# rohithr87/CILRS-Autonomous-Driving-CARLA

Measured on AMD Instinct MI355X. Metric: frames/sec CILRS train batch=128, higher is better.
Workload: dtype f32; 1 GPU; CILRS ResNet-34 train step (fwd+loss+bwd+Adam), Config A, 200x88 RGB, B=128/GPU, fp32; global_batch=128, parallelism=single

## Files before the change

### cilrs-autonomous-driving-carla_amd/cilrs_mi355/_lib.py

```python
from __future__ import annotations

import ctypes as C
import os

_HERE = os.path.dirname(os.path.abspath(__file__))
LIB_PATH = os.environ.get("CILRS_LIB") or os.path.join(_HERE, "libcilrs_hip.so")

c_float_p = C.POINTER(C.c_float)
vp = C.c_void_p
sz = C.c_size_t
i32 = C.c_int
i64 = C.c_int64
f32 = C.c_float
f64 = C.c_double
u64 = C.c_uint64


class Buffers(C.Structure):
    _fields_ = [("params", vp), ("grads", vp), ("bn_running", vp), ("bn_nbt", vp),
                ("workspace", vp)]


class AdamArgs(C.Structure):
    _fields_ = [("exp_avg", vp), ("exp_avg_sq", vp), ("lr", C.c_double), ("beta1", C.c_double),
# ... 112 lines not shown
                                         f32, vp, f32, vp]),
    "cilrs_swap": (i32, [vp, vp, sz, vp]),
    "cilrs_augment_u8": (i32, [vp, vp, i32, i32, i32, vp, vp, vp]),
    "cilrs_batch_assemble": (i32, [vp, i64, vp, vp, vp, vp, vp, i32, i32, i32, vp, vp, vp, vp, vp,
                                   vp]),
    "cilrs_eval_acc_doubles": (i32, []),
    "cilrs_eval_accumulate": (i32, [vp, vp, vp, vp, vp, i32, vp, vp, vp]),
    "cilrs_net_profile_enable": (i32, [vp, i32]),
    "cilrs_net_profile_collect": (i32, [vp]),
    "cilrs_net_profile_count": (i32, [vp]),
    "cilrs_net_profile_entry": (i32, [vp, i32, C.c_char_p, i32, C.POINTER(C.c_longlong),
                                      C.POINTER(f64), C.POINTER(f64), C.POINTER(f64)]),
    "cilrs_net_profile_reset": (i32, [vp]),
    "cilrs_conv2d_fwd": (i32, [vp, vp, vp] + [i32] * 11 + [vp, sz, vp]),
    "cilrs_conv2d_dgrad": (i32, [vp, vp, vp, vp] + [i32] * 11 + [vp, sz, vp]),
    "cilrs_conv2d_wgrad_scratch_floats": (sz, [i32] * 9),
    "cilrs_conv2d_wgrad": (i32, [vp, vp, vp, vp] + [i32] * 10 + [vp]),
    "cilrs_conv2d_16_scratch_halfs": (sz, [i32] * 8),
    "cilrs_conv2d_fwd_16": (i32, [vp, vp, vp, vp] + [i32] * 9 + [vp, vp]),
    "cilrs_conv2d_dgrad_16": (i32, [vp, vp, vp, vp] + [i32] * 9 + [vp, vp]),
    "cilrs_conv2d_wgrad_16_scratch_floats": (sz, [i32] * 8),
    "cilrs_conv2d_wgrad_16": (i32, [vp, vp, vp, vp] + [i32] * 9 + [vp, vp]),
    "cilrs_conv2d_train_16": (i32, [vp] * 9 + [i32, vp] + [i32] * 12 + [vp, vp]),
    "cilrs_conv2d_infer_16": (i32, [vp] * 5 + [i32] * 11 + [vp]),
    "cilrs_stem_fold_16": (i32, [vp, vp, vp, vp, i32, vp]),
    "cilrs_stem_infer_16": (i32, [vp, vp, vp, vp, i32, i32, i32, i32, vp]),
    "cilrs_maxpool_infer_16": (i32, [vp, vp, i32, i32, i32, i32, i32, vp]),
    "cilrs_avgpool_infer_16": (i32, [vp, vp, i32, i32, i32, i32, i32, vp]),
    "cilrs_bn16_train_fwd": (i32, [vp, i32, i32, vp, vp, vp, vp, vp, C.c_float, C.c_float, vp, i32,
                                   vp, vp, vp, i32, vp]),
# ... 70 lines not shown
```

### cilrs-autonomous-driving-carla_amd/csrc/common.h

```cpp
#pragma once
#include <hip/hip_runtime.h>
#include <stdint.h>
#include <stddef.h>
#include "../../include/cilrs_hip.h"

namespace cilrs {

typedef float f32x4 __attribute__((ext_vector_type(4)));
typedef float f32x16 __attribute__((ext_vector_type(16)));

void set_error(const char* fmt, ...);
const char* last_error();

#define CILRS_CHECK(cond, ...)                   \
    do {                                         \
        if (!(cond)) {                           \
            ::cilrs::set_error(__VA_ARGS__);     \
            return 1;                            \
        }                                        \
    } while (0)

#define CILRS_HIP(expr)                                                                 \
    do {                                                                                \
        hipError_t e_ = (expr);                                                         \
// ... 17 lines not shown
static inline int cdiv(int a, int b) { return (a + b - 1) / b; }

int device_cus();
int set_max_dynamic_lds(const void* kernel, int bytes);

constexpr float kImageMean[3] = {0.485f, 0.456f, 0.406f};
constexpr float kImageStd[3] = {0.229f, 0.224f, 0.225f};

#ifdef CILRS_EXPERIMENTS
int experiment_env(const char* name, int dflt);
#else
static inline int experiment_env(const char*, int dflt) { return dflt; }
#endif
static inline size_t cdivz(size_t a, size_t b) { return (a + b - 1) / b; }

struct ConvMulti {
    int n;
    int tile_begin[5];
    int Ho[4], Wo[4], out_h0[4], out_w0[4], ntaps[4];
    int tap_dh[4][4], tap_dw[4][4], tap_w[4][4];
};

struct ConvArgs {
    const float* x;
    const float* w;
    float* y;
    const float* addend;
    const float* bias;
    const float* ch_scale;
    const float* ch_shift;
    int relu_post;
    const float* mask;
    int N, H, W, Cin;
    int Ho, Wo, Cout;
    int KH, KW;
// ... 7 lines not shown
    int ntaps;
    int tap_dh[16], tap_dw[16], tap_w[16];
    float* bn_partial;
    int* bn_nblk;
    const float* bwd_z; const float* bwd_y; const float* bwd_stats; int bwd_relu;
    float* bwd_partial; int* bwd_nblk;
    float* scratch;
    size_t scratch_floats;
    int force_cfg;
    int force_splitk;
    int splitk;
    int prio_mode;
    ConvMulti multi;
};
int launch_conv_igemm(const ConvArgs& a, hipStream_t s);
int slab_reduce_rows(int M, int C, int* rows_per_block);
int launch_slab_reduce_cols(int mode, const float* slabs, int splits, float* y, const float* addend,
                            int M, int C, const float* bwd_z, const float* bwd_y,
                            const float* bwd_stats, int bwd_relu, float* partial, hipStream_t s);
struct DgradArgs {
    const float* dy; const float* w; float* dx; const float* addend;
    const float* mask; int mask_ld; float mask_scale;
    int N, H, W, Cin, Ho, Wo, Cout, K, stride, pad;
    int dy_ld, dx_ld;
    float* scratch; size_t scratch_floats; int force_cfg, force_splitk;
    const float* bwd_z; const float* bwd_y; const float* bwd_stats; int bwd_relu;
    float* bwd_partial; int* bwd_nblk;
};
int launch_conv_dgrad(const DgradArgs& a, hipStream_t s);

// ... 496 lines not shown
```

### cilrs-autonomous-driving-carla_amd/csrc/conv_igemm.hip

```cpp
#include "common.h"

#include <stdlib.h>
#include <string.h>

namespace cilrs {

namespace {

constexpr int BK = 32;
constexpr int APITCH = BK + 4;

__device__ float g_zero_page[64];

__device__ __forceinline__ int xcd_remap(int bid, int nwg) {
    const int q = nwg >> 3, r = nwg & 7, xcd = bid & 7;
    const int base = xcd < r ? xcd * (q + 1) : r * (q + 1) + (xcd - r) * q;
    return base + (bid >> 3);
}

#ifndef CILRS_IGEMM_DBG
#define CILRS_IGEMM_DBG 0
#endif
template <int BM, int BN, bool TAP_UNIFORM, bool DMA>
constexpr bool igemm_swz() { return DMA || (BM == 64 && BN == 64 && TAP_UNIFORM); }
// ... 15 lines not shown
    constexpr int JQ = BN / 4, BROWS = 256 / JQ;

    extern __shared__ __attribute__((aligned(16))) float smem[];
    float* As = smem;
    float* Bs = smem + NSTAGE * BM * APIT;

    const int tid = threadIdx.x;
    const int lane = tid & 63, wave = tid >> 6;
    const int l31 = lane & 31, lh = lane >> 5;
    const int wm = wave / WN, wn = wave % WN;

    wave_priority(a.prio_mode < 16 ? a.prio_mode : 0);
    wave_stagger(a.prio_mode);
    const int tilesN = a.Cout / BN;
    int logical = xcd_remap(blockIdx.x, gridDim.x);
    int cls = 0;
    int P_Ho = a.Ho, P_Wo = a.Wo, P_h0 = a.out_h0, P_w0 = a.out_w0, P_ntaps = a.ntaps;
    int M = M_, KT = KT_;
    if constexpr (MULTI) {
        while (cls + 1 < a.multi.n && logical >= a.multi.tile_begin[cls + 1]) ++cls;
        logical -= a.multi.tile_begin[cls];
        P_Ho = a.multi.Ho[cls]; P_Wo = a.multi.Wo[cls];
        P_h0 = a.multi.out_h0[cls]; P_w0 = a.multi.out_w0[cls];
        P_ntaps = a.multi.ntaps[cls];
        M = a.N * P_Ho * P_Wo;
        KT = P_ntaps * (a.Cin / BK);
    }
    auto tap_dh = [&](int t) { if constexpr (MULTI) return a.multi.tap_dh[cls][t]; else return a.tap_dh[t]; };
    auto tap_dw = [&](int t) { if constexpr (MULTI) return a.multi.tap_dw[cls][t]; else return a.tap_dw[t]; };
    auto tap_w = [&](int t) { if constexpr (MULTI) return a.multi.tap_w[cls][t]; else return a.tap_w[t]; };
    const int m0 = (logical / tilesN) * BM;
    const int n0 = (logical % tilesN) * BN;

    int kt_begin = 0, kt_end = KT;
    if (a.splitk > 1) {
        const int per = (KT + a.splitk - 1) / a.splitk;
        kt_begin = blockIdx.z * per;
        kt_end = min(KT, kt_begin + per);
    }
    const int nt = max(kt_end - kt_begin, 0);

    const int kq = tid & 7, r0 = tid >> 3;
    const int kql = DMA ? (kq ^ ((r0 >> 1) & 7)) : kq;
    long rowBase[A_PASSES];
    unsigned rowMask[A_PASSES];
    int rowH[A_PASSES], rowW[A_PASSES];
    const int HoWo = P_Ho * P_Wo;
#pragma unroll
    for (int i = 0; i < A_PASSES; ++i) {
        const int m = m0 + r0 + 32 * i;
        rowMask[i] = 0u; rowBase[i] = 0; rowH[i] = -(1 << 20); rowW[i] = 0;
        if (m < M) {
            const int n = m / HoWo, rem = m - n * HoWo;
// ... 307 lines not shown
            s1 += __shfl_xor(s1, 32);
            s2 += __shfl_xor(s2, 32);
            if (lh == 0) {
                red[(wm * BN + wn * WTN + j * 32 + l31) * 2] = s1;
                red[(wm * BN + wn * WTN + j * 32 + l31) * 2 + 1] = s2;
            }
        }
        __syncthreads();
        if (tid < BN) {
            float t1 = 0.f, t2 = 0.f;
#pragma unroll
            for (int w = 0; w < WM; ++w) {
                t1 += red[(w * BN + tid) * 2];
                t2 += red[(w * BN + tid) * 2 + 1];
            }
            const size_t mt = (size_t)(logical / tilesN), nmt = (size_t)((M + BM - 1) / BM);
            a.bn_partial[(size_t)(n0 + tid) * nmt + mt] = t1;
            a.bn_partial[(size_t)(a.Cout + n0 + tid) * nmt + mt] = t2;
        }
    }

    const bool partial = a.splitk > 1;
    const bool dense = (a.out_sh == 1) && (a.out_sw == 1) && (a.out_H == P_Ho) &&
                       (a.out_W == P_Wo);
    float* yout = partial ? a.y + (size_t)blockIdx.z * M * a.y_ld : a.y;
    const bool bwd_red = a.bwd_partial != nullptr && !partial;
    float bs1[TN], bs2[TN];
#pragma unroll
    for (int j = 0; j < TN; ++j) { bs1[j] = 0.f; bs2[j] = 0.f; }
#pragma unroll
    for (int i = 0; i < TM; ++i) {
#pragma unroll
        for (int j = 0; j < TN; ++j) {
            const int co = n0 + wn * WTN + j * 32 + l31;
            const int mbase = m0 + wm * WTM + i * 32 + 4 * lh;
            int pix[16];
#pragma unroll
            for (int r = 0; r < 16; ++r) {
                const int m = min(mbase + (r & 3) + 8 * (r >> 2), M - 1);
                if (dense || partial) {
                    pix[r] = m;
                } else {
                    const int n = m / HoWo, rem = m - n * HoWo;
                    const int oh = rem / P_Wo, ow = rem - oh * P_Wo;
                    pix[r] = (n * a.out_H + oh * a.out_sh + P_h0) * a.out_W +
                             ow * a.out_sw + P_w0;
                }
            }
            float v[16];
#pragma unroll
            for (int r = 0; r < 16; ++r) v[r] = acc[i][j][r];
            if (!partial) {
                if (a.ch_scale) {
                    const float sc = a.ch_scale[co], sh = a.ch_shift[co];
#pragma unroll
// ... 58 lines not shown
            float s1 = bs1[j] + __shfl_xor(bs1[j], 32);
            float s2 = bs2[j] + __shfl_xor(bs2[j], 32);
            if (lh == 0) {
                red[(wm * BN + wn * WTN + j * 32 + l31) * 2] = s1;
                red[(wm * BN + wn * WTN + j * 32 + l31) * 2 + 1] = s2;
            }
        }
        __syncthreads();
        if (tid < BN) {
            float t1 = 0.f, t2 = 0.f;
#pragma unroll
            for (int w = 0; w < WM; ++w) {
                t1 += red[(w * BN + tid) * 2];
                t2 += red[(w * BN + tid) * 2 + 1];
            }
            const size_t mt = (size_t)(logical / tilesN), nmt = (size_t)((M + BM - 1) / BM);
            a.bwd_partial[(size_t)(n0 + tid) * nmt + mt] = t1;
            a.bwd_partial[(size_t)(a.Cout + n0 + tid) * nmt + mt] = t2;
        }
    }
}

__device__ __forceinline__ int out_pixel(const ConvArgs& a, int m, int HoWo) {
    const int n = m / HoWo, rem = m - n * HoWo;
    const int oh = rem / a.Wo, ow = rem - oh * a.Wo;
    return (n * a.out_H + oh * a.out_sh + a.out_h0) * a.out_W + ow * a.out_sw + a.out_w0;
}

template <int MODE>
__global__ __launch_bounds__(256) void splitk_reduce_cols_kernel(const ConvArgs a,
                                                                 const float* __restrict__ part,
// ... 217 lines not shown
    CILRS_LAUNCH_CHECK();
    return 0;
}

struct Cfg { int bm, bn, occ; bool dma; float rate[5]; };
const Cfg kCfg[6] = {
    {128, 128, 2, false, {100.f, 113.f, 0.f, 0.f}},
    {128, 64, 2, false, {81.f, 100.f, 0.f, 0.f}},
    {64, 64, 5, false, {64.f, 90.f, 101.f, 108.f, 112.f}},
    {128, 128, 1, true, {125.f, 0.f, 0.f, 0.f}},
    {128, 64, 2, true, {110.f, 121.f, 0.f, 0.f}},
    {64, 64, 3, true, {94.f, 106.f, 111.f, 0.f}},
};
constexpr int kNumCfg = 6;

double cfg_cost(int M, int Cout, int KT, const Cfg& c, int splitk) {
    if (Cout % c.bn) return 1e30;
    const double blocks = (double)cdiv(M, c.bm) * (Cout / c.bn) * splitk;
    const long per_cu = (long)((blocks + 255) / 256);
    const double ktiles = (double)cdiv(KT, splitk);
    const double unit = 2.0 * c.bm * c.bn * BK * ktiles;
    const long full = per_cu / c.occ, rem = per_cu % c.occ;
    double t = 0.0;
    if (full) t += full * unit * 256.0 * c.occ / (c.rate[c.occ - 1] * 1e6);
    if (rem) t += unit * 256.0 * rem / (c.rate[rem - 1] * 1e6);
    t += (full + (rem ? 1 : 0)) * 2.5;
    if (splitk > 1) t += 3.0 + 0.12 * splitk + (double)M * Cout * 4.0 * (splitk + 1) / 3.0e6;
    return t;
}

struct Choice { int cfg; int splitk; };

Choice choose(int M, int Cout, int KT, bool allow_split, int force_cfg, int force_splitk) {
    static const int splits[11] = {1, 2, 3, 4, 6, 8, 12, 16, 24, 32, 48};
    static const int use_dma = experiment_env("CILRS_IGEMM_DMA", 0);
    Choice best{2, 1};
    double bc = 1e30;
    for (int c = 0; c < kNumCfg; ++c) {
        if (force_cfg >= 0 && c != force_cfg) continue;
        if (force_cfg < 0 && use_dma == 0 && kCfg[c].dma) continue;
        if (force_cfg < 0 && use_dma == 2 && !kCfg[c].dma) continue;
        for (int si = 0; si < 11; ++si) {
            int sk = splits[si];
            if (force_splitk > 0) {
                if (si > 0) break;
                sk = force_splitk;
            } else if (sk > 1 && (!allow_split || KT < 2 * sk)) {
                continue;
            }
            const double cost = cfg_cost(M, Cout, KT, kCfg[c], sk);
            if (cost < bc) { bc = cost; best = {c, sk}; }
        }
    }
    return best;
}

}

int launch_conv_igemm(const ConvArgs& a_in, hipStream_t s) {
    ConvArgs a = a_in;
    a.prio_mode = wave_priority_mode();
    const int M = a.N * a.Ho * a.Wo;
    const bool uniform = (a.Cin % BK) == 0;
    CILRS_CHECK(!uniform || ((size_t)a.N * a.H * a.W * a.x_ld * sizeof(float) < (1ull << 32) &&
                             (size_t)(a.w_mode == 0 ? a.Cout : a.Cin) * a.KH * a.KW *
                                     (a.w_mode == 0 ? a.Cin : a.w_cin) * sizeof(float) < (1ull << 32)),
                "conv_igemm: tensor larger than 4 GB");
    if (a.out_H == 0) {
        a.out_H = a.Ho; a.out_W = a.Wo; a.out_sh = a.out_sw = 1; a.out_h0 = a.out_w0 = 0;
    }
    if (uniform && a.ntaps == 0) {
        CILRS_CHECK(a.KH * a.KW <= 16, "conv_igemm: more than 16 taps on the uniform path");
        a.ntaps = a.KH * a.KW;
        for (int t = 0; t < a.ntaps; ++t) {
            a.tap_dh[t] = t / a.KW;
            a.tap_dw[t] = t % a.KW;
            a.tap_w[t] = (a.w_mode == 0) ? t : a.ntaps - 1 - t;
        }
    }
    const int KT = uniform ? a.ntaps * (a.Cin / BK) : cdiv(a.KH * a.KW * a.Cin, BK);
    const int Krow = a.KH * a.KW * a.Cin;
    CILRS_CHECK(a.Cout % 64 == 0, "conv_igemm: Cout=%d must be a multiple of 64", a.Cout);
    CILRS_CHECK(a.Cin % 4 == 0 && a.x_ld % 4 == 0 && a.y_ld % 4 == 0,
                "conv_igemm: Cin/x_ld/y_ld must be multiples of 4 (%d,%d,%d)", a.Cin, a.x_ld,
                a.y_ld);
    CILRS_CHECK(uniform || a.w_mode == 0, "conv_igemm: the generic-tap path is forward-only");
    CILRS_CHECK(a.w_mode == 0 || a.w_cin % 4 == 0, "conv_igemm: w_cin must be a multiple of 4");
    CILRS_CHECK(((uintptr_t)a.x & 15) == 0 && ((uintptr_t)a.w & 15) == 0 &&
                    ((uintptr_t)a.y & 15) == 0,
                "conv_igemm: pointers must be 16-byte aligned");
    CILRS_CHECK(M > 0 && (size_t)a.N * a.H * a.W < (1u << 31), "conv_igemm: bad M");
    CILRS_CHECK(a.ntaps <= 16, "conv_igemm: too many taps");

    const size_t slab = (size_t)M * a.y_ld;
    const bool can_split = a.scratch != nullptr && a.scratch_floats >= 2 * slab && uniform;
    Choice ch = choose(M, a.Cout, KT, can_split, a.force_cfg, a.force_splitk);
    while (ch.splitk > 1 && (size_t)ch.splitk * slab > a.scratch_floats) --ch.splitk;
    CILRS_CHECK(ch.splitk == 1 || (a.scratch && uniform), "conv_igemm: split-K needs scratch");
    CILRS_CHECK(ch.cfg >= 0 && ch.cfg < kNumCfg && a.Cout % kCfg[ch.cfg].bn == 0,
                "conv_igemm: tile config %d does not fit Cout=%d", ch.cfg, a.Cout);
    a.splitk = ch.splitk;
    const bool dense_out = a.out_sh == 1 && a.out_sw == 1 && a.out_H == a.Ho && a.out_W == a.Wo;
    const int tpr = a.Cout >> 2;
    const bool cols_ok = a.splitk > 1 && dense_out && a.Cout % 4 == 0 && tpr <= 256 &&
                         256 % tpr == 0 && a.y_ld % 4 == 0 && (!a.mask || a.mask_ld % 4 == 0);
    int cols_rows = 0, cols_nblk = 0;
    if (cols_ok && (a.bn_partial || a.bwd_partial)) {
        const int rpi = 256 / tpr;
        cols_rows = cdiv(cdiv(M, 1024), rpi) * rpi;
        cols_nblk = cdiv(M, cols_rows);
    }
    float* const fwd_partial = a.bn_partial;
    float* const bwd_partial = a.bwd_partial;
    if (a_in.bn_nblk)
        *a_in.bn_nblk = !a.bn_partial ? 0
                        : a.splitk == 1 ? cdiv(M, kCfg[ch.cfg].bm) : cols_nblk;
    if (!(a.splitk == 1 && dense_out)) a.bwd_partial = nullptr;
    if (a_in.bwd_nblk)
        *a_in.bwd_nblk = a.bwd_partial ? cdiv(M, kCfg[ch.cfg].bm) : (bwd_partial ? cols_nblk : 0);
    float* final_y = a.y;
    if (a.splitk > 1) a.y = a.scratch;

    int rc = 1;
#define CILRS_DISPATCH(BM_, BN_, DMA_)                                                          \
    do {                                                                                        \
        if (a.w_mode == 1) rc = launch_cfg<BM_, BN_, 2, 2, true, 1, DMA_>(a, M, Krow, KT, s);   \
        else if (uniform)  rc = launch_cfg<BM_, BN_, 2, 2, true, 0, DMA_>(a, M, Krow, KT, s);   \
        else               rc = launch_cfg<BM_, BN_, 2, 2, false, 0, DMA_>(a, M, Krow, KT, s);  \
    } while (0)
    switch (ch.cfg) {
        case 0: CILRS_DISPATCH(128, 128, false); break;
        case 1: CILRS_DISPATCH(128, 64, false); break;
        case 2: CILRS_DISPATCH(64, 64, false); break;
        case 3: CILRS_DISPATCH(128, 128, true); break;
        case 4: CILRS_DISPATCH(128, 64, true); break;
        default: CILRS_DISPATCH(64, 64, true); break;
    }
#undef CILRS_DISPATCH
// ... 103 lines not shown
        ConvMulti& mu = c.multi;
        memset(&mu, 0, sizeof(mu));
        mu.n = ncl;
        const int tilesN = c.Cout / 64;
        int total = 0;
        for (int i = 0; i < ncl; ++i) {
            mu.tile_begin[i] = total;
            total += cdiv(c.N * cl[i].Ho * cl[i].Wo, 64) * tilesN;
            mu.Ho[i] = cl[i].Ho; mu.Wo[i] = cl[i].Wo;
            mu.out_h0[i] = cl[i].ph; mu.out_w0[i] = cl[i].pw; mu.ntaps[i] = cl[i].nt;
            for (int t = 0; t < cl[i].nt; ++t) {
                mu.tap_dh[i][t] = cl[i].dh[t]; mu.tap_dw[i][t] = cl[i].dw[t];
                mu.tap_w[i][t] = cl[i].tw[t];
            }
        }
        for (int i = ncl; i < 5; ++i) mu.tile_begin[i] = total;
        CILRS_CHECK((size_t)c.N * c.H * c.W * c.x_ld * sizeof(float) < (1ull << 32) &&
                        (size_t)c.Cin * c.KH * c.KW * c.w_cin * sizeof(float) < (1ull << 32),
                    "conv_dgrad: tensor larger than 4 GB");
        CILRS_CHECK(((uintptr_t)c.x & 15) == 0 && ((uintptr_t)c.w & 15) == 0 &&
                        ((uintptr_t)c.y & 15) == 0 && c.x_ld % 4 == 0 && c.y_ld % 4 == 0 &&
                        c.w_cin % 4 == 0,
                    "conv_dgrad: operands must be 16-byte aligned");
        constexpr size_t lds = (size_t)(2 * 64 * BK + 2 * BK * 64) * sizeof(float);
        if (set_max_dynamic_lds(
                reinterpret_cast<const void*>(&conv_igemm_kernel<64, 64, 2, 2, true, 1, false, true>),
                (int)lds))
            return 1;
        conv_igemm_kernel<64, 64, 2, 2, true, 1, false, true>
            <<<dim3(total, 1, 1), 256, lds, s>>>(c, 0, c.KH * c.KW * c.Cin, 0);
        CILRS_LAUNCH_CHECK();
        return 0;
    }
    for (int ph = 0; ph < 2; ++ph)
        for (int pw = 0; pw < 2; ++pw) {
            ConvArgs c = a;
            c.Ho = (d.H - ph + 1) / 2; c.Wo = (d.W - pw + 1) / 2;
            if (c.Ho <= 0 || c.Wo <= 0) continue;
            c.stride = 1; c.pad = 0;
            c.out_H = d.H; c.out_W = d.W; c.out_sh = 2; c.out_sw = 2; c.out_h0 = ph; c.out_w0 = pw;
            int nt = 0;
            for (int kh = 0; kh < d.K; ++kh) {
                if ((ph + d.pad - kh) & 1) continue;
                for (int kw = 0; kw < d.K; ++kw) {
                    if ((pw + d.pad - kw) & 1) continue;
                    c.tap_dh[nt] = (ph + d.pad - kh) / 2;
                    c.tap_dw[nt] = (pw + d.pad - kw) / 2;
// ... 20 lines not shown
```

### cilrs-autonomous-driving-carla_amd/csrc/net.hip

```cpp
#include "common.h"
#include "../../include/cilrs_hip.h"

#include <math.h>
#include <stdarg.h>
#include <stdio.h>
#include <stdlib.h>
#include <string.h>

#include <algorithm>
#include <map>
#include <mutex>
#include <set>
#include <string>
#include <vector>

namespace cilrs {

static thread_local char g_err[1024] = "";
void set_error(const char* fmt, ...) {
    va_list ap;
    va_start(ap, fmt);
    vsnprintf(g_err, sizeof(g_err), fmt, ap);
    va_end(ap);
}
// ... 878 lines not shown
        WgradArgs wa;
        memset(&wa, 0, sizeof(wa));
        wa.N = B; wa.H = wa.W = wa.Ho = wa.Wo = 1; wa.Cin = comb; wa.Cout = 256;
        wa.KH = wa.KW = 1; wa.stride = 1;
        const size_t sf = wgrad_scratch_floats(wa);
        if (sf > slabs_max) slabs_max = sf;
    }
    (void)feat;
    if (!trainable) gmax = 4;
    n->gmax = gmax;
    for (int i = 0; i < kNumG; ++i) n->G[i] = bump.take(gmax);
    {
        size_t need = bn_partial_floats(512);
        if (trainable)
            for (size_t ci = 0; ci < A.convs.size(); ++ci) {
                const size_t t = (size_t)cdiv(n->cg[ci].M, 64) * 2 * A.convs[ci].cout;
                if (t > need) need = t;
                const size_t tb = (size_t)cdiv(B * n->cg[ci].H * n->cg[ci].W, 64) * 2 *
                                  A.convs[ci].cin;
                if (ci > 0 && tb > need) need = tb;
                if (bn_partial_floats(A.convs[ci].cout) > need)
                    need = bn_partial_floats(A.convs[ci].cout);
            }
        n->bn_partial = bump.take(need);
        n->bn_partial2 = bump.take(need);
    }
    n->bn_coef = bump.take(5 * 2048);
    n->slabs_floats = slabs_max;
    n->slabs = bump.take(slabs_max > 0 ? slabs_max : 4);
    n->ksplit_floats = ksplit_max;
    n->ksplit = bump.take(ksplit_max > 0 ? ksplit_max : 4);
    n->status_b = bump.take(64) * sizeof(float);
    CILRS_CHECK((int)A.convs.size() <= kMaxConvs, "too many convolutions for the BN tables");
// ... 2299 lines not shown
                       int force_cfg, int force_splitk, float* scratch, size_t scratch_floats,
                       void* stream) {
    CILRS_CHECK(KH == KW, "dgrad: square kernels only");
    DgradArgs a;
    memset(&a, 0, sizeof(a));
    a.dy = dy; a.w = w; a.dx = dx; a.addend = addend;
    a.N = N; a.H = H; a.W = W; a.Cin = Cin;
    a.Ho = (H + 2 * pad - KH) / stride + 1; a.Wo = (W + 2 * pad - KW) / stride + 1;
    a.Cout = Cout; a.K = KH; a.stride = stride; a.pad = pad;
    a.dy_ld = Cout; a.dx_ld = Cin;
    a.scratch = scratch; a.scratch_floats = scratch_floats;
    a.force_cfg = force_cfg; a.force_splitk = force_splitk;
    return launch_conv_dgrad(a, reinterpret_cast<hipStream_t>(stream));
}

static WgradArgs make_wgrad(const float* x, const float* dy, float* dw, float* scratch, int N,
                            int H, int W, int Cin, int Cout, int KH, int KW, int stride, int pad,
                            int Cin_dst) {
    WgradArgs a;
    memset(&a, 0, sizeof(a));
    a.x = x; a.dy = dy; a.dw = dw; a.slabs = scratch;
    a.N = N; a.H = H; a.W = W; a.Cin = Cin;
    a.Ho = (H + 2 * pad - KH) / stride + 1; a.Wo = (W + 2 * pad - KW) / stride + 1; a.Cout = Cout;
    a.KH = KH; a.KW = KW; a.stride = stride; a.pad = pad;
    a.x_ld = Cin; a.dy_ld = Cout; a.Cin_dst = Cin_dst; a.accumulate = 0;
    return a;
}

size_t cilrs_conv2d_wgrad_scratch_floats(int N, int H, int W, int Cin, int Cout, int KH, int KW,
                                         int stride, int pad) {
// ... 351 lines not shown
```

### include/cilrs_hip.h

```cpp
#ifndef CILRS_HIP_H
#define CILRS_HIP_H

#include <stddef.h>
#include <stdint.h>

#ifdef __cplusplus
extern "C" {
#endif

typedef struct cilrs_net cilrs_net;

int cilrs_version(void);
const char* cilrs_last_error(void);

int cilrs_num_params(void);
int cilrs_num_bn(void);
size_t cilrs_param_arena_floats(void);
size_t cilrs_param_count(void);
int cilrs_param_info(int i, char* name, int name_cap, size_t* offset, size_t* numel, int* ndim,
                     int* shape4);
int cilrs_bn_info(int j, char* prefix, int prefix_cap, int* channels, size_t* rm_offset,
                  size_t* rv_offset);
size_t cilrs_bn_arena_floats(void);

// ... 264 lines not shown
int cilrs_net_profile_enable(cilrs_net* net, int on);
int cilrs_net_profile_collect(cilrs_net* net);
int cilrs_net_profile_count(const cilrs_net* net);
int cilrs_net_profile_entry(const cilrs_net* net, int i, char* label, int label_cap,
                            long long* calls, double* total_ms, double* total_flops,
                            double* total_bytes);
int cilrs_net_profile_reset(cilrs_net* net);

int cilrs_conv2d_fwd(const float* x, const float* w, float* y, int N, int H, int W, int Cin,
                     int Cout, int KH, int KW, int stride, int pad, int force_cfg,
                     int force_splitk, float* scratch, size_t scratch_floats, void* stream);
int cilrs_conv2d_dgrad(const float* dy, const float* w, float* dx, const float* addend, int N,
                       int H, int W, int Cin, int Cout, int KH, int KW, int stride, int pad,
                       int force_cfg, int force_splitk, float* scratch, size_t scratch_floats,
                       void* stream);
size_t cilrs_conv2d_wgrad_scratch_floats(int N, int H, int W, int Cin, int Cout, int KH, int KW,
                                         int stride, int pad);
int cilrs_conv2d_wgrad(const float* x, const float* dy, float* dw, float* scratch, int N, int H,
                       int W, int Cin, int Cout, int KH, int KW, int stride, int pad,
                       int Cin_dst, void* stream);

size_t cilrs_conv2d_16_scratch_halfs(int N, int H, int W, int Cin, int Cout, int K, int stride,
                                     int pad);
int cilrs_conv2d_fwd_16(const float* x, const float* w, float* y, float* bn_partial, int N, int H,
                        int W, int Cin, int Cout, int K, int stride, int pad, int bf16,
                        void* scratch16, void* stream);
int cilrs_conv2d_dgrad_16(const float* dy, const float* w, float* dx, const float* addend, int N,
                          int H, int W, int Cin, int Cout, int K, int stride, int pad, int bf16,
                          void* scratch16, void* stream);
size_t cilrs_conv2d_wgrad_16_scratch_floats(int N, int H, int W, int Cin, int Cout, int K,
// ... 98 lines not shown
```

Measured before the change: 14120 frames/s.

## Split padded stride-1 convs into border position classes to skip padding taps

Extends the multi-class implicit-GEMM path to ordinary forward and dgrad stride-1 convolutions. The output is partitioned into position classes (interior, edges, corners), and each class iterates only the taps that land inside the image, so no MACs are spent on zero padding. A cost model decides when this beats the single-launch kernel, and split-K ranges plus BN partial-stat indexing are remapped for the per-class tile layout. It is on by default through an env flag. The cost is more launch metadata, corner classes with fewer taps that can leave tiles imbalanced, and larger BN partial buffers.

```diff
diff --git a/cilrs-autonomous-driving-carla_amd/cilrs_mi355/_lib.py b/cilrs-autonomous-driving-carla_amd/cilrs_mi355/_lib.py
--- a/cilrs-autonomous-driving-carla_amd/cilrs_mi355/_lib.py
+++ b/cilrs-autonomous-driving-carla_amd/cilrs_mi355/_lib.py
@@ -150,6 +150,11 @@
     "cilrs_net_profile_reset": (i32, [vp]),
     "cilrs_conv2d_fwd": (i32, [vp, vp, vp] + [i32] * 11 + [vp, sz, vp]),
     "cilrs_conv2d_dgrad": (i32, [vp, vp, vp, vp] + [i32] * 11 + [vp, sz, vp]),
+    "cilrs_conv2d_fwd_stats": (i32, [vp, vp, vp, vp, C.POINTER(i32)] + [i32] * 10 + [vp, sz, vp]),
+    "cilrs_conv2d_dgrad_bnbwd": (i32, [vp] * 7 + [i32, vp, C.POINTER(i32)] + [i32] * 10
+                                 + [vp, sz, vp]),
+    "cilrs_conv2d_takes_classes": (i32, [i32] * 9 + [sz, i32]),
+    "cilrs_net_conv_classes": (i32, [vp, i32, C.POINTER(i32), C.POINTER(i32)]),
     "cilrs_conv2d_wgrad_scratch_floats": (sz, [i32] * 9),
     "cilrs_conv2d_wgrad": (i32, [vp, vp, vp, vp] + [i32] * 10 + [vp]),
     "cilrs_conv2d_16_scratch_halfs": (sz, [i32] * 8),
diff --git a/cilrs-autonomous-driving-carla_amd/csrc/common.h b/cilrs-autonomous-driving-carla_amd/csrc/common.h
--- a/cilrs-autonomous-driving-carla_amd/csrc/common.h
+++ b/cilrs-autonomous-driving-carla_amd/csrc/common.h
@@ -55,11 +55,15 @@
 #endif
 static inline size_t cdivz(size_t a, size_t b) { return (a + b - 1) / b; }
 
+constexpr int kConvMultiMax = 9;
 struct ConvMulti {
     int n;
-    int tile_begin[5];
-    int Ho[4], Wo[4], out_h0[4], out_w0[4], ntaps[4];
-    int tap_dh[4][4], tap_dw[4][4], tap_w[4][4];
+    int spread;
+    int tile_begin[kConvMultiMax + 1];
+    int Ho[kConvMultiMax], Wo[kConvMultiMax], out_h0[kConvMultiMax], out_w0[kConvMultiMax];
+    int ntaps[kConvMultiMax];
+    short tap_dh[kConvMultiMax][kConvMultiMax], tap_dw[kConvMultiMax][kConvMultiMax];
+    short tap_w[kConvMultiMax][kConvMultiMax];
 };
 
 struct ConvArgs {
@@ -97,6 +101,8 @@
     ConvMulti multi;
 };
 int launch_conv_igemm(const ConvArgs& a, hipStream_t s);
+bool conv_igemm_takes_classes(int N, int H, int W, int Cin, int Cout, int K, int stride, int pad,
+                              bool dgrad, size_t scratch_floats, int force_splitk = 0);
 int slab_reduce_rows(int M, int C, int* rows_per_block);
 int launch_slab_reduce_cols(int mode, const float* slabs, int splits, float* y, const float* addend,
                             int M, int C, const float* bwd_z, const float* bwd_y,
diff --git a/cilrs-autonomous-driving-carla_amd/csrc/conv_igemm.hip b/cilrs-autonomous-driving-carla_amd/csrc/conv_igemm.hip
--- a/cilrs-autonomous-driving-carla_amd/csrc/conv_igemm.hip
+++ b/cilrs-autonomous-driving-carla_amd/csrc/conv_igemm.hip
@@ -53,12 +53,17 @@
     wave_stagger(a.prio_mode);
     const int tilesN = a.Cout / BN;
     int logical = xcd_remap(blockIdx.x, gridDim.x);
+    if constexpr (MULTI) {
+        if (a.multi.spread) logical = blockIdx.x;
+    }
     int cls = 0;
     int P_Ho = a.Ho, P_Wo = a.Wo, P_h0 = a.out_h0, P_w0 = a.out_w0, P_ntaps = a.ntaps;
     int M = M_, KT = KT_;
+    int mt_base = 0;
     if constexpr (MULTI) {
         while (cls + 1 < a.multi.n && logical >= a.multi.tile_begin[cls + 1]) ++cls;
         logical -= a.multi.tile_begin[cls];
+        mt_base = a.multi.tile_begin[cls] / tilesN;
         P_Ho = a.multi.Ho[cls]; P_Wo = a.multi.Wo[cls];
         P_h0 = a.multi.out_h0[cls]; P_w0 = a.multi.out_w0[cls];
         P_ntaps = a.multi.ntaps[cls];
@@ -73,9 +78,20 @@
 
     int kt_begin = 0, kt_end = KT;
     if (a.splitk > 1) {
-        const int per = (KT + a.splitk - 1) / a.splitk;
-        kt_begin = blockIdx.z * per;
-        kt_end = min(KT, kt_begin + per);
+        if constexpr (MULTI) {
+            const int ct = a.Cin / BK, lo = (int)blockIdx.z * KT_, hi = lo + KT_;
+            int b = 0, e = 0;
+            for (int t = 0; t < P_ntaps; ++t) {
+                const int pos = (W_MODE == 0) ? tap_w(t) : a.KH * a.KW - 1 - tap_w(t);
+                b += min(max(lo - pos * ct, 0), ct);
+                e += min(max(hi - pos * ct, 0), ct);
+            }
+            kt_begin = b; kt_end = e;
+        } else {
+            const int per = (KT + a.splitk - 1) / a.splitk;
+            kt_begin = blockIdx.z * per;
+            kt_end = min(KT, kt_begin + per);
+        }
     }
     const int nt = max(kt_end - kt_begin, 0);
 
@@ -413,7 +429,9 @@
                 t1 += red[(w * BN + tid) * 2];
                 t2 += red[(w * BN + tid) * 2 + 1];
             }
-            const size_t mt = (size_t)(logical / tilesN), nmt = (size_t)((M + BM - 1) / BM);
+            const size_t mt = (size_t)(mt_base + logical / tilesN);
+            const size_t nmt = MULTI ? (size_t)(a.multi.tile_begin[a.multi.n] / tilesN)
+                                     : (size_t)((M + BM - 1) / BM);
             a.bn_partial[(size_t)(n0 + tid) * nmt + mt] = t1;
             a.bn_partial[(size_t)(a.Cout + n0 + tid) * nmt + mt] = t2;
         }
@@ -422,7 +440,8 @@
     const bool partial = a.splitk > 1;
     const bool dense = (a.out_sh == 1) && (a.out_sw == 1) && (a.out_H == P_Ho) &&
                        (a.out_W == P_Wo);
-    float* yout = partial ? a.y + (size_t)blockIdx.z * M * a.y_ld : a.y;
+    const bool slab_rows = partial && !MULTI;
+    float* yout = partial ? a.y + (size_t)blockIdx.z * (MULTI ? M_ : M) * a.y_ld : a.y;
     const bool bwd_red = a.bwd_partial != nullptr && !partial;
     float bs1[TN], bs2[TN];
 #pragma unroll
@@ -437,7 +456,7 @@
 #pragma unroll
             for (int r = 0; r < 16; ++r) {
                 const int m = min(mbase + (r & 3) + 8 * (r >> 2), M - 1);
-                if (dense || partial) {
+                if (dense || slab_rows) {
                     pix[r] = m;
                 } else {
                     const int n = m / HoWo, rem = m - n * HoWo;
@@ -526,7 +545,9 @@
                 t1 += red[(w * BN + tid) * 2];
                 t2 += red[(w * BN + tid) * 2 + 1];
             }
-            const size_t mt = (size_t)(logical / tilesN), nmt = (size_t)((M + BM - 1) / BM);
+            const size_t mt = (size_t)(mt_base + logical / tilesN);
+            const size_t nmt = MULTI ? (size_t)(a.multi.tile_begin[a.multi.n] / tilesN)
+                                     : (size_t)((M + BM - 1) / BM);
             a.bwd_partial[(size_t)(n0 + tid) * nmt + mt] = t1;
             a.bwd_partial[(size_t)(a.Cout + n0 + tid) * nmt + mt] = t2;
         }
@@ -774,11 +795,8 @@
 };
 constexpr int kNumCfg = 6;
 
-double cfg_cost(int M, int Cout, int KT, const Cfg& c, int splitk) {
-    if (Cout % c.bn) return 1e30;
-    const double blocks = (double)cdiv(M, c.bm) * (Cout / c.bn) * splitk;
+double cfg_cost_blocks(double blocks, double ktiles, int M, int Cout, const Cfg& c, int splitk) {
     const long per_cu = (long)((blocks + 255) / 256);
-    const double ktiles = (double)cdiv(KT, splitk);
     const double unit = 2.0 * c.bm * c.bn * BK * ktiles;
     const long full = per_cu / c.occ, rem = per_cu % c.occ;
     double t = 0.0;
@@ -787,6 +805,11 @@
     t += (full + (rem ? 1 : 0)) * 2.5;
     if (splitk > 1) t += 3.0 + 0.12 * splitk + (double)M * Cout * 4.0 * (splitk + 1) / 3.0e6;
     return t;
+}
+double cfg_cost(int M, int Cout, int KT, const Cfg& c, int splitk) {
+    if (Cout % c.bn) return 1e30;
+    const double blocks = (double)cdiv(M, c.bm) * (Cout / c.bn) * splitk;
+    return cfg_cost_blocks(blocks, (double)cdiv(KT, splitk), M, Cout, c, splitk);
 }
 
 struct Choice { int cfg; int splitk; };
@@ -815,6 +838,163 @@
     return best;
 }
 
+bool classes_enabled() {
+    static const int env = getenv("CILRS_IGEMM_CLASSES") ? atoi(getenv("CILRS_IGEMM_CLASSES")) : 1;
+    return env != 0;
+}
+bool classes_spread() {
+    static const int chunks = experiment_env("CILRS_IGEMM_CLASS_CHUNKS", 0);
+    return chunks == 0;
+}
+
+struct TapRun { int begin, len; unsigned taps; };
+int position_runs(int out, int in, int K, int pad, TapRun (&r)[3]) {
+    int n = 0;
+    for (int o = 0; o < out; ++o) {
+        unsigned m = 0u;
+        for (int k = 0; k < K; ++k) {
+            const int i = o - pad + k;
+            if (i >= 0 && i < in) m |= 1u << k;
+        }
+        if (m == 0u) return 0;
+        if (n > 0 && r[n - 1].taps == m) { ++r[n - 1].len; continue; }
+        if (n == 3) return 0;
+        r[n++] = TapRun{o, 1, m};
+    }
+    return n;
+}
+
+int build_position_classes(const ConvArgs& a, ConvMulti& mu) {
+    if (a.stride != 1 || a.pad <= 0 || a.ntaps > kConvMultiMax || a.KH * a.KW != a.ntaps ||
+        a.Cout % 64 != 0 || a.H >= 32768 || a.W >= 32768)
+        return 0;
+    TapRun rr[3], rc[3];
+    const int nr = position_runs(a.Ho, a.H, a.KH, a.pad, rr);
+    const int nc = position_runs(a.Wo, a.W, a.KW, a.pad, rc);
+    if (nr == 0 || nc == 0 || nr * nc < 2) return 0;
+    struct Cls { int h0, w0, Ho, Wo, nt; short dh[kConvMultiMax], dw[kConvMultiMax], tw[kConvMultiMax]; };
+    Cls cl[kConvMultiMax];
+    int ncl = 0;
+    for (int i = 0; i < nr; ++i)
+        for (int j = 0; j < nc; ++j) {
+            Cls k;
+            k.h0 = rr[i].begin; k.w0 = rc[j].begin; k.Ho = rr[i].len; k.Wo = rc[j].len; k.nt = 0;
+            if ((long)a.N * k.Ho * k.Wo < 64) return 0;
+            for (int t = 0; t < a.ntaps; ++t) {
+                if (!((rr[i].taps >> a.tap_dh[t]) & 1u) || !((rc[j].taps >> a.tap_dw[t]) & 1u))
+                    continue;
+                k.dh[k.nt] = (short)(k.h0 - a.pad + a.tap_dh[t]);
+                k.dw[k.nt] = (short)(k.w0 - a.pad + a.tap_dw[t]);
+                k.tw[k.nt] = (short)a.tap_w[t];
+                ++k.nt;
+            }
+            cl[ncl++] = k;
+        }
+    for (int i = 1; i < ncl; ++i)
+        for (int j = i; j > 0 && cl[j].nt > cl[j - 1].nt; --j) {
+            const Cls t = cl[j]; cl[j] = cl[j - 1]; cl[j - 1] = t;
+        }
+    memset(&mu, 0, sizeof(mu));
+    mu.n = ncl;
+    mu.spread = classes_spread() ? 1 : 0;
+    const int tilesN = a.Cout / 64;
+    int total = 0;
+    for (int i = 0; i < ncl; ++i) {
+        mu.tile_begin[i] = total;
+        total += cdiv(a.N * cl[i].Ho * cl[i].Wo, 64) * tilesN;
+        mu.Ho[i] = cl[i].Ho; mu.Wo[i] = cl[i].Wo;
+        mu.out_h0[i] = cl[i].h0; mu.out_w0[i] = cl[i].w0; mu.ntaps[i] = cl[i].nt;
+        for (int t = 0; t < cl[i].nt; ++t) {
+            mu.tap_dh[i][t] = cl[i].dh[t]; mu.tap_dw[i][t] = cl[i].dw[t];
+            mu.tap_w[i][t] = cl[i].tw[t];
+        }
+    }
+    for (int i = ncl; i <= kConvMultiMax; ++i) mu.tile_begin[i] = total;
+    return total;
+}
+
+int choose_classes(const ConvArgs& a, int M, int sk, double single_cost, ConvMulti& mu) {
+    const int tiles = build_position_classes(a, mu);
+    if (tiles == 0) return 0;
+    if ((long)tiles * sk > 256L * kCfg[2].occ) return 0;
+    double sum = 0.0;
+    for (int c = 0; c < mu.n; ++c)
+        sum += (double)(mu.tile_begin[c + 1] - mu.tile_begin[c]) * mu.ntaps[c] * (a.Cin / BK);
+    const double cost =
+        cfg_cost_blocks((double)tiles * sk, sum / ((double)tiles * sk), M, a.Cout, kCfg[2], sk);
+    return cost < single_cost ? tiles : 0;
+}
+
+struct IgemmPlan { Choice ch; int class_tiles; };
+IgemmPlan plan_igemm(const ConvArgs& a, bool class_candidate, ConvMulti& mu) {
+    const int M = a.N * a.Ho * a.Wo;
+    const bool uniform = (a.Cin % BK) == 0;
+    const int KT = uniform ? a.ntaps * (a.Cin / BK) : cdiv(a.KH * a.KW * a.Cin, BK);
+    const size_t slab = (size_t)M * a.y_ld;
+    const bool can_split = a.scratch != nullptr && a.scratch_floats >= 2 * slab && uniform;
+    IgemmPlan p;
+    p.ch = choose(M, a.Cout, KT, can_split, a.force_cfg, a.force_splitk);
+    while (p.ch.splitk > 1 && (size_t)p.ch.splitk * slab > a.scratch_floats) --p.ch.splitk;
+    p.class_tiles = 0;
+    if (class_candidate && uniform && (a.force_cfg == -1 || a.force_cfg == 2) && classes_enabled() &&
+        p.ch.cfg == 2) {
+        const double single = cfg_cost(M, a.Cout, KT, kCfg[2], p.ch.splitk);
+        p.class_tiles = choose_classes(a, M, p.ch.splitk, single, mu);
+    }
+    return p;
+}
+
+void dense_taps(ConvArgs& a) {
+    a.ntaps = a.KH * a.KW;
+    for (int t = 0; t < a.ntaps; ++t) {
+        a.tap_dh[t] = t / a.KW;
+        a.tap_dw[t] = t % a.KW;
+        a.tap_w[t] = (a.w_mode == 0) ? t : a.ntaps - 1 - t;
+    }
+}
+
+static_assert(sizeof(ConvArgs) + 3 * sizeof(int) <= 4096, "kernel arguments exceed the launch limit");
+template <int W_MODE>
+int launch_multi(const ConvArgs& a, int tiles, int M_all, int kt_per_split, hipStream_t s) {
+    constexpr size_t lds = (size_t)(2 * 64 * BK + 2 * BK * 64) * sizeof(float);
+    if (set_max_dynamic_lds(
+            reinterpret_cast<const void*>(&conv_igemm_kernel<64, 64, 2, 2, true, W_MODE, false, true>),
+            (int)lds))
+        return 1;
+    conv_igemm_kernel<64, 64, 2, 2, true, W_MODE, false, true>
+        <<<dim3(tiles, 1, a.splitk > 1 ? a.splitk : 1), 256, lds, s>>>(a, M_all,
+                                                                      a.KH * a.KW * a.Cin,
+                                                                      kt_per_split);
+    CILRS_LAUNCH_CHECK();
+    return 0;
+}
+
+}
+
+bool conv_igemm_takes_classes(int N, int H, int W, int Cin, int Cout, int K, int stride, int pad,
+                              bool dgrad, size_t scratch_floats, int force_splitk) {
+    if (stride != 1 || K * K > 16 || Cin <= 0 || Cout <= 0) return false;
+    const int Ho = H + 2 * pad - K + 1, Wo = W + 2 * pad - K + 1;
+    if (Ho <= 0 || Wo <= 0) return false;
+    ConvArgs a;
+    memset(&a, 0, sizeof(a));
+    a.N = N; a.KH = a.KW = K; a.stride = 1;
+    if (!dgrad) {
+        a.H = H; a.W = W; a.Cin = Cin; a.Ho = Ho; a.Wo = Wo; a.Cout = Cout; a.pad = pad;
+        a.w_mode = 0; a.w_cin = Cin;
+    } else {
+        a.H = Ho; a.W = Wo; a.Cin = Cout; a.Ho = H; a.Wo = W; a.Cout = Cin; a.pad = K - 1 - pad;
+        a.w_mode = 1; a.w_cin = Cin;
+    }
+    if (a.Cin % BK != 0 || a.Cout % 64 != 0) return false;
+    a.x_ld = a.Cin; a.y_ld = a.Cout;
+    a.force_cfg = -1; a.force_splitk = force_splitk;
+    a.scratch_floats = scratch_floats;
+    a.scratch = scratch_floats ? reinterpret_cast<float*>(sizeof(float) * 4) : nullptr;
+    a.out_H = a.Ho; a.out_W = a.Wo; a.out_sh = a.out_sw = 1;
+    dense_taps(a);
+    ConvMulti mu;
+    return plan_igemm(a, true, mu).class_tiles > 0;
 }
 
 int launch_conv_igemm(const ConvArgs& a_in, hipStream_t s) {
@@ -822,6 +1002,7 @@
     a.prio_mode = wave_priority_mode();
     const int M = a.N * a.Ho * a.Wo;
     const bool uniform = (a.Cin % BK) == 0;
+    const bool class_candidate = a_in.out_H == 0 && a_in.ntaps == 0 && a_in.multi.n == 0;
     CILRS_CHECK(!uniform || ((size_t)a.N * a.H * a.W * a.x_ld * sizeof(float) < (1ull << 32) &&
                              (size_t)(a.w_mode == 0 ? a.Cout : a.Cin) * a.KH * a.KW *
                                      (a.w_mode == 0 ? a.Cin : a.w_cin) * sizeof(float) < (1ull << 32)),
@@ -831,12 +1012,7 @@
     }
     if (uniform && a.ntaps == 0) {
         CILRS_CHECK(a.KH * a.KW <= 16, "conv_igemm: more than 16 taps on the uniform path");
-        a.ntaps = a.KH * a.KW;
-        for (int t = 0; t < a.ntaps; ++t) {
-            a.tap_dh[t] = t / a.KW;
-            a.tap_dw[t] = t % a.KW;
-            a.tap_w[t] = (a.w_mode == 0) ? t : a.ntaps - 1 - t;
-        }
+        dense_taps(a);
     }
     const int KT = uniform ? a.ntaps * (a.Cin / BK) : cdiv(a.KH * a.KW * a.Cin, BK);
     const int Krow = a.KH * a.KW * a.Cin;
@@ -852,10 +1028,10 @@
     CILRS_CHECK(M > 0 && (size_t)a.N * a.H * a.W < (1u << 31), "conv_igemm: bad M");
     CILRS_CHECK(a.ntaps <= 16, "conv_igemm: too many taps");
 
-    const size_t slab = (size_t)M * a.y_ld;
-    const bool can_split = a.scratch != nullptr && a.scratch_floats >= 2 * slab && uniform;
-    Choice ch = choose(M, a.Cout, KT, can_split, a.force_cfg, a.force_splitk);
-    while (ch.splitk > 1 && (size_t)ch.splitk * slab > a.scratch_floats) --ch.splitk;
+    const IgemmPlan plan = plan_igemm(a, class_candidate, a.multi);
+    const Choice ch = plan.ch;
+    const int class_tiles = plan.class_tiles;
+    if (class_tiles == 0) a.multi.n = 0;
     CILRS_CHECK(ch.splitk == 1 || (a.scratch && uniform), "conv_igemm: split-K needs scratch");
     CILRS_CHECK(ch.cfg >= 0 && ch.cfg < kNumCfg && a.Cout % kCfg[ch.cfg].bn == 0,
                 "conv_igemm: tile config %d does not fit Cout=%d", ch.cfg, a.Cout);
@@ -872,16 +1048,24 @@
     }
     float* const fwd_partial = a.bn_partial;
     float* const bwd_partial = a.bwd_partial;
+    const int mtiles = class_tiles > 0 ? class_tiles / (a.Cout / 64) : cdiv(M, kCfg[ch.cfg].bm);
     if (a_in.bn_nblk)
-        *a_in.bn_nblk = !a.bn_partial ? 0
-                        : a.splitk == 1 ? cdiv(M, kCfg[ch.cfg].bm) : cols_nblk;
+        *a_in.bn_nblk = !a.bn_partial ? 0 : a.splitk == 1 ? mtiles : cols_nblk;
     if (!(a.splitk == 1 && dense_out)) a.bwd_partial = nullptr;
     if (a_in.bwd_nblk)
-        *a_in.bwd_nblk = a.bwd_partial ? cdiv(M, kCfg[ch.cfg].bm) : (bwd_partial ? cols_nblk : 0);
+        *a_in.bwd_nblk = a.bwd_partial ? mtiles : (bwd_partial ? cols_nblk : 0);
     float* final_y = a.y;
     if (a.splitk > 1) a.y = a.scratch;
 
     int rc = 1;
+    if (class_tiles > 0) {
+        const int pad = a.pad;
+        a.pad = 0;
+        const int per = cdiv(KT, a.splitk > 1 ? a.splitk : 1);
+        rc = a.w_mode == 1 ? launch_multi<1>(a, class_tiles, M, per, s)
+                           : launch_multi<0>(a, class_tiles, M, per, s);
+        a.pad = pad;
+    } else
 #define CILRS_DISPATCH(BM_, BN_, DMA_)                                                          \
     do {                                                                                        \
         if (a.w_mode == 1) rc = launch_cfg<BM_, BN_, 2, 2, true, 1, DMA_>(a, M, Krow, KT, s);   \
@@ -1015,7 +1199,7 @@
                 mu.tap_w[i][t] = cl[i].tw[t];
             }
         }
-        for (int i = ncl; i < 5; ++i) mu.tile_begin[i] = total;
+        for (int i = ncl; i <= kConvMultiMax; ++i) mu.tile_begin[i] = total;
         CILRS_CHECK((size_t)c.N * c.H * c.W * c.x_ld * sizeof(float) < (1ull << 32) &&
                         (size_t)c.Cin * c.KH * c.KW * c.w_cin * sizeof(float) < (1ull << 32),
                     "conv_dgrad: tensor larger than 4 GB");
@@ -1023,15 +1207,7 @@
                         ((uintptr_t)c.y & 15) == 0 && c.x_ld % 4 == 0 && c.y_ld % 4 == 0 &&
                         c.w_cin % 4 == 0,
                     "conv_dgrad: operands must be 16-byte aligned");
-        constexpr size_t lds = (size_t)(2 * 64 * BK + 2 * BK * 64) * sizeof(float);
-        if (set_max_dynamic_lds(
-                reinterpret_cast<const void*>(&conv_igemm_kernel<64, 64, 2, 2, true, 1, false, true>),
-                (int)lds))
-            return 1;
-        conv_igemm_kernel<64, 64, 2, 2, true, 1, false, true>
-            <<<dim3(total, 1, 1), 256, lds, s>>>(c, 0, c.KH * c.KW * c.Cin, 0);
-        CILRS_LAUNCH_CHECK();
-        return 0;
+        return launch_multi<1>(c, total, c.N * d.H * d.W, 0, s);
     }
     for (int ph = 0; ph < 2; ++ph)
         for (int pw = 0; pw < 2; ++pw) {
diff --git a/cilrs-autonomous-driving-carla_amd/csrc/net.hip b/cilrs-autonomous-driving-carla_amd/csrc/net.hip
--- a/cilrs-autonomous-driving-carla_amd/csrc/net.hip
+++ b/cilrs-autonomous-driving-carla_amd/csrc/net.hip
@@ -916,9 +916,9 @@
         size_t need = bn_partial_floats(512);
         if (trainable)
             for (size_t ci = 0; ci < A.convs.size(); ++ci) {
-                const size_t t = (size_t)cdiv(n->cg[ci].M, 64) * 2 * A.convs[ci].cout;
+                const size_t t = (size_t)(cdiv(n->cg[ci].M, 64) + kConvMultiMax) * 2 * A.convs[ci].cout;
                 if (t > need) need = t;
-                const size_t tb = (size_t)cdiv(B * n->cg[ci].H * n->cg[ci].W, 64) * 2 *
+                const size_t tb = (size_t)(cdiv(B * n->cg[ci].H * n->cg[ci].W, 64) + kConvMultiMax) * 2 *
                                   A.convs[ci].cin;
                 if (ci > 0 && tb > need) need = tb;
                 if (bn_partial_floats(A.convs[ci].cout) > need)
@@ -3248,6 +3248,71 @@
     return launch_conv_dgrad(a, reinterpret_cast<hipStream_t>(stream));
 }
 
+int cilrs_conv2d_fwd_stats(const float* x, const float* w, float* y, float* partial, int* nblk,
+                           int N, int H, int W, int Cin, int Cout, int K, int stride, int pad,
+                           int force_cfg, int force_splitk, float* scratch, size_t scratch_floats,
+                           void* stream) {
+    CILRS_CHECK(x && w && y && partial && nblk, "conv2d_fwd_stats: NULL argument");
+    ConvArgs a;
+    memset(&a, 0, sizeof(a));
+    a.x = x; a.w = w; a.y = y;
+    a.N = N; a.H = H; a.W = W; a.Cin = Cin;
+    a.Ho = (H + 2 * pad - K) / stride + 1; a.Wo = (W + 2 * pad - K) / stride + 1; a.Cout = Cout;
+    a.KH = a.KW = K; a.stride = stride; a.pad = pad;
+    a.x_ld = Cin; a.y_ld = Cout; a.w_mode = 0; a.w_cin = Cin;
+    a.scratch = scratch; a.scratch_floats = scratch_floats;
+    a.force_cfg = force_cfg; a.force_splitk = force_splitk;
+    a.bn_partial = partial; a.bn_nblk = nblk; *nblk = 0;
+    CILRS_CHECK((size_t)(cdiv(N * a.Ho * a.Wo, 64) + kConvMultiMax) * 2 * Cout <= bn_partial_floats(Cout),
+                "conv2d_fwd_stats: more than %zu rows", bn_partial_floats(Cout) / 2 / Cout * 64);
+    return launch_conv_igemm(a, reinterpret_cast<hipStream_t>(stream));
+}
+
+int cilrs_conv2d_dgrad_bnbwd(const float* dy, const float* w, float* dx, const float* addend,
+                             const float* bwd_z, const float* bwd_y, const float* bwd_stats,
+                             int bwd_relu, float* partial, int* nblk, int N, int H, int W, int Cin,
+                             int Cout, int K, int stride, int pad, int force_cfg, int force_splitk,
+                             float* scratch, size_t scratch_floats, void* stream) {
+    CILRS_CHECK(dy && w && dx && bwd_y && bwd_stats && partial && nblk && (bwd_z || !bwd_relu),
+                "conv2d_dgrad_bnbwd: NULL argument");
+    CILRS_CHECK(stride == 1, "conv2d_dgrad_bnbwd: stride 1 only");
+    DgradArgs a;
+    memset(&a, 0, sizeof(a));
+    a.dy = dy; a.w = w; a.dx = dx; a.addend = addend;
+    a.N = N; a.H = H; a.W = W; a.Cin = Cin;
+    a.Ho = H + 2 * pad - K + 1; a.Wo = W + 2 * pad - K + 1;
+    a.Cout = Cout; a.K = K; a.stride = stride; a.pad = pad;
+    a.dy_ld = Cout; a.dx_ld = Cin;
+    a.scratch = scratch; a.scratch_floats = scratch_floats;
+    a.force_cfg = force_cfg; a.force_splitk = force_splitk;
+    a.bwd_z = bwd_z; a.bwd_y = bwd_y; a.bwd_stats = bwd_stats; a.bwd_relu = bwd_relu;
+    a.bwd_partial = partial; a.bwd_nblk = nblk; *nblk = 0;
+    CILRS_CHECK((size_t)(cdiv(N * H * W, 64) + kConvMultiMax) * 2 * Cin <= bn_partial_floats(Cin),
+                "conv2d_dgrad_bnbwd: more than %zu rows", bn_partial_floats(Cin) / 2 / Cin * 64);
+    return launch_conv_dgrad(a, reinterpret_cast<hipStream_t>(stream));
+}
+
+int cilrs_conv2d_takes_classes(int N, int H, int W, int Cin, int Cout, int K, int stride, int pad,
+                               int dgrad, size_t scratch_floats, int force_splitk) {
+    return conv_igemm_takes_classes(N, H, W, Cin, Cout, K, stride, pad, dgrad != 0, scratch_floats,
+                                    force_splitk) ? 1 : 0;
+}
+
+int cilrs_net_conv_classes(const cilrs_net* net, int conv, int* fwd, int* dgrad) {
+    CILRS_CHECK(net != nullptr, "conv_classes: net is NULL");
+    CILRS_CHECK(conv >= 0 && conv < (int)net->cg.size(), "conv_classes: conv %d out of range", conv);
+    const ConvT& c = net->A->convs[conv];
+    const ConvG& g = net->cg[conv];
+    const bool igemm = conv > 0 && !net->wino_on[conv] && !net->bf16_train;
+    const bool yes_f = igemm && conv_igemm_takes_classes(net->B, g.H, g.W, c.cin, c.cout, c.k, c.stride,
+                                                         c.pad, false, net->ksplit_floats);
+    const bool yes_d = igemm && conv_igemm_takes_classes(net->B, g.H, g.W, c.cin, c.cout, c.k, c.stride,
+                                                         c.pad, true, net->ksplit_floats);
+    if (fwd) *fwd = yes_f ? 1 : 0;
+    if (dgrad) *dgrad = yes_d ? 1 : 0;
+    return 0;
+}
+
 static WgradArgs make_wgrad(const float* x, const float* dy, float* dw, float* scratch, int N,
                             int H, int W, int Cin, int Cout, int KH, int KW, int stride, int pad,
                             int Cin_dst) {
diff --git a/include/cilrs_hip.h b/include/cilrs_hip.h
--- a/include/cilrs_hip.h
+++ b/include/cilrs_hip.h
@@ -302,6 +302,18 @@
                        int H, int W, int Cin, int Cout, int KH, int KW, int stride, int pad,
                        int force_cfg, int force_splitk, float* scratch, size_t scratch_floats,
                        void* stream);
+int cilrs_conv2d_fwd_stats(const float* x, const float* w, float* y, float* partial, int* nblk,
+                           int N, int H, int W, int Cin, int Cout, int K, int stride, int pad,
+                           int force_cfg, int force_splitk, float* scratch, size_t scratch_floats,
+                           void* stream);
+int cilrs_conv2d_dgrad_bnbwd(const float* dy, const float* w, float* dx, const float* addend,
+                             const float* bwd_z, const float* bwd_y, const float* bwd_stats,
+                             int bwd_relu, float* partial, int* nblk, int N, int H, int W, int Cin,
+                             int Cout, int K, int stride, int pad, int force_cfg, int force_splitk,
+                             float* scratch, size_t scratch_floats, void* stream);
+int cilrs_conv2d_takes_classes(int N, int H, int W, int Cin, int Cout, int K, int stride, int pad,
+                               int dgrad, size_t scratch_floats, int force_splitk);
+int cilrs_net_conv_classes(const cilrs_net* net, int conv, int* fwd, int* dgrad);
 size_t cilrs_conv2d_wgrad_scratch_floats(int N, int H, int W, int Cin, int Cout, int KH, int KW,
                                          int stride, int pad);
 int cilrs_conv2d_wgrad(const float* x, const float* dy, float* dw, float* scratch, int N, int H,
```

New measurement: 14280 frames/s (median of 6 runs). 1.1% higher.
